# Excalibur1224/Cuda-v-MPI

Hardware: AMD Instinct MI355X
Metric: Riemann subintervals/sec at N=1e9 fp64; |error| vs analytic π (higher is better)
Workload: dtype fp64

## Files before the change

csrc/include/miint/integrands.hpp:

```cpp
#pragma once

#include <hip/hip_runtime.h>

#include "miint/common.hpp"
#include "miint/fast_trig.hpp"

namespace miint {

template <class D>
struct TileDefaults {
  template <DivMode M>
  __host__ __device__ static constexpr int tile_len() { return 32; }
  template <int U, DivMode M>
  __device__ static constexpr double anchor() { return 0.0; }
  template <int U, DivMode M>
  __device__ __forceinline__ double tile_acc(double x0, double h, double acc) const {
    return acc + static_cast<const D*>(this)->template tile<U, M>(x0, h);
  }
};

struct Pi4 : TileDefaults<Pi4> {
  static constexpr double kScale = 4.0;
  static constexpr int kPairs = 16;
  static constexpr int kSub = 2 * kPairs;
  static constexpr int kSubs = 12;
  static constexpr int kSeriesTile = kSub * kSubs;
  static constexpr double kSumK2 = (kSeriesTile / 2) * (kSeriesTile / 2 - 1) * (kSeriesTile - 1) / 3.0 +
                                   (kSeriesTile / 2) * (kSeriesTile / 2 - 1) + kSeriesTile / 4.0;
  static_assert(kSumK2 == 4718560.0, "sum of squared midpoint offsets of a 384-sample tile");

  template <DivMode M>
  __host__ __device__ static constexpr int tile_len() {
    return (M == DivMode::kSeries || M == DivMode::kSeriesExact) ? kSeriesTile : 32;
  }

  static constexpr double kMeanK2 = 85.25;
  static constexpr int kPk2Sgpr = 5;
  double pk[kPairs];
  double pk2[kPairs];
  double pc[kSubs / 2];
  double pcm[kSubs / 2];
  double c15;
  typedef float f32x2 __attribute__((ext_vector_type(2)));
  f32x2 pkf[kPairs];

  __device__ __forceinline__ static double opaque_s(double v) {
    asm volatile("" : "+s"(v));
    return v;
  }
  __device__ __forceinline__ static double opaque_v(double v) {
    asm volatile("" : "+v"(v));
    return v;
  }
  template <bool K2 = true>
  __device__ __forceinline__ void init() {
#pragma unroll
    for (int j = 0; j < kPairs; ++j) {
      pk[j] = opaque_s(j + 0.5);
      const double k2 = (j + 0.5) * (j + 0.5) - kMeanK2;
      if constexpr (K2) {
        pk2[j] = j < kPk2Sgpr ? opaque_s(k2) : opaque_v(k2);
      } else {
        pk2[j] = k2;
        const f32x2 kk = {j + 0.5f, -(j + 0.5f)};
        pkf[j] = __builtin_bit_cast(f32x2, opaque_s(__builtin_bit_cast(double, kk)));
      }
    }
#pragma unroll
    for (int i = 0; i < kSubs / 2; ++i) {
      const double c0 = kSub * (i + 0.5);
      pc[i] = opaque_s(c0);
      pcm[i] = opaque_s(c0 + kMeanK2 / c0);
    }
    c15 = opaque_s(1.5);
  }

  __device__ __forceinline__ double point(double x) const { return 1.0 / fma(x, x, 1.0); }

  __device__ __forceinline__ static double recip_narrow(double d) {
    double r = __builtin_amdgcn_rcp(d);
    r = fma(r, fma(-d, r, 1.0), r);
    r = fma(r, fma(-d, r, 1.0), r);
    return fma(fma(-d, r, 1.0), r, r);
  }

  struct Seed {
    double s, em, a, b;
  };
  __device__ __forceinline__ static Seed seed(double xm, double h) {
    const double dm = fma(xm, xm, 1.0);
    double s = __builtin_amdgcn_rcp(dm);
    s = fma(s, fma(-dm, s, 1.0), s);
    return {s, fma(-dm, s, 1.0), (-2.0 * h) * xm * s, -(h * h) * s};
  }
  __device__ __forceinline__ Seed seed_half(double xm, double h) const {
    const double dm = fma(xm, xm, 1.0);
    const double s = __builtin_amdgcn_rcp(dm);
    return {s, fma(-dm, s, c15), (-2.0 * h) * xm * s, -(h * h) * s};
  }
  __device__ __forceinline__ static double side(const double* t, int q) {
    return q < kSubs / 2 ? -t[kSubs / 2 - 1 - q] : t[q - kSubs / 2];
  }
  __device__ __forceinline__ double centre_g(const Seed& sd, int q) const {
    return fma(side(pc, q), fma(side(pcm, q), sd.b, sd.a), sd.em);
  }
  __device__ __forceinline__ double centre_slope(const Seed& sd, double b2, int q) const {
    return fma(side(pc, q), b2, sd.a);
  }

  template <int U, DivMode M>
  __device__ __forceinline__ double tile(double x0, double h) const {
    static_assert(U % 2 == 0, "pair evaluation needs an even tile");
    static_assert(M != DivMode::kSeries, "kSeries runs through tile_acc");
    if constexpr (M == DivMode::kIeee) {
      double acc = 0.0;
#pragma unroll
      for (int u = 0; u < U; ++u) {
        const double x = fma(static_cast<double>(u), h, x0);
        acc += recip_narrow(fma(x, x, 1.0));
      }
      return acc;
    } else {
      const Seed sd = seed(fma(0.5 * (U - 1), h, x0), h);
      double t1a = 0.0, t1b = 0.0, t2 = 0.0;
#pragma unroll
      for (int u = 0; u < U; u += 2) {
        const double xa = fma(static_cast<double>(u), h, x0);
        const double xb = fma(static_cast<double>(u + 1), h, x0);
        const double ea = fma(-fma(xa, xa, 1.0), sd.s, 1.0);
        const double eb = fma(-fma(xb, xb, 1.0), sd.s, 1.0);
        t1a += ea;
        t1b += eb;
        t2 = fma(ea, ea, t2);
        t2 = fma(eb, eb, t2);
      }
      return fma(sd.s, (t1a + t1b) + t2, static_cast<double>(U) * sd.s);
    }
  }

  template <int U, DivMode M>
  __device__ static constexpr double anchor() {
    return (M == DivMode::kSeries || M == DivMode::kSeriesExact) ? 0.5 * (U - 1) : 0.0;
  }

  __device__ __forceinline__ Seed seed_exact(double xm, double h) const {
    const double dm = fma(xm, xm, 1.0);
    const double s = __builtin_amdgcn_rcp(dm);
    const double q = xm * s;
    const double qe = fma(xm, s, -q);
    const double em = fma(-xm, qe, fma(-xm, q, 1.0 - s));
    return {s, em, (-2.0 * h) * xm * s, -(h * h) * s};
  }

  template <int U, DivMode M>
  __device__ __forceinline__ double tile_acc(double xa, double h, double acc) const {
    if constexpr (M == DivMode::kSeries) {
      static_assert(U == kSeriesTile, "series tiles are kSubs sub-tiles of kSub samples");
      const Seed sd = seed_half(xa, h);
      const double b2 = 2.0 * sd.b;
      double t = 0.75 * U;
#pragma unroll
      for (int q = 0; q < kSubs; ++q) {
        const double eh = centre_g(sd, q);
        const double a = centre_slope(sd, b2, q);
#pragma unroll
        for (int j = 0; j < kPairs; ++j) {
          const double c = fma(pk2[j], sd.b, eh);
          const double gp = fma(pk[j], a, c);
          const double gn = fma(-pk[j], a, c);
          t = fma(gp, gp, t);
          t = fma(gn, gn, t);
          asm volatile("" : "+v"(t));
        }
      }
      return fma(sd.s, t, acc);
    } else if constexpr (M == DivMode::kSeriesExact) {
      static_assert(U == kSeriesTile, "series tiles are kSubs sub-tiles of kSub samples");
      const Seed sd = seed_exact(xa, h);
      const double b2 = 2.0 * sd.b;
      const double lin = fma(kSumK2, sd.b, static_cast<double>(U) * sd.em);
      f32x2 t2 = {0.0f, 0.0f};
#pragma unroll
      for (int q = 0; q < kSubs; ++q) {
        const f32x2 ec = static_cast<float>(centre_g(sd, q));
        const f32x2 a = static_cast<float>(centre_slope(sd, b2, q));
#pragma unroll
        for (int j = 0; j < kPairs; ++j) {
          const f32x2 e = __builtin_elementwise_fma(pkf[j], a, ec);
          t2 = __builtin_elementwise_fma(e, e, t2);
          asm volatile("" : "+v"(t2));
        }
      }
      const double t = lin + (static_cast<double>(t2.x) + static_cast<double>(t2.y));
      return fma(sd.s, t, fma(sd.s, static_cast<double>(U), acc));
    } else {
      return acc + tile<U, M>(xa, h);
    }
  }

  __device__ __forceinline__ double series_exact_point(double xm, double h, int u) const {
    const Seed sd = seed_exact(xm, h);
    const double b2 = 2.0 * sd.b;
    const int q = u / kSub, w = u % kSub;
    const double ec = centre_g(sd, q);
    const double a = centre_slope(sd, b2, q);
    const int j = w >= kSub / 2 ? w - kSub / 2 : kSub / 2 - 1 - w;
    const double kj = w >= kSub / 2 ? pk[j] : -pk[j];
    const double e = fma(kj, a, fma(fma(kj, kj, -kMeanK2), sd.b, ec));
    const float e_sq = fmaf(static_cast<float>(kj), static_cast<float>(a), static_cast<float>(ec));
    const float sq = e_sq * e_sq;
    return fma(sd.s, e + static_cast<double>(sq), sd.s);
  }

  __device__ __forceinline__ double series_point(double xm, double h, int u) const {
    const Seed sd = seed_half(xm, h);
    const double b2 = 2.0 * sd.b;
    const int q = u / kSub, w = u % kSub;
    const double eh = centre_g(sd, q);
    const double a = centre_slope(sd, b2, q);
    const int j = w >= kSub / 2 ? w - kSub / 2 : kSub / 2 - 1 - w;
    const double c = fma(pk2[j], sd.b, eh);
    const double g = w >= kSub / 2 ? fma(pk[j], a, c) : fma(-pk[j], a, c);
    return sd.s * fma(g, g, 0.75);
  }
};

struct Pi4Wide : TileDefaults<Pi4Wide> {
  static constexpr double kScale = 4.0;
  __device__ __forceinline__ double point(double x) const { return 1.0 / fma(x, x, 1.0); }
  template <int U, DivMode M>
  __device__ __forceinline__ double tile(double x0, double h) const {
    static_assert(M == DivMode::kIeee, "wide-domain Pi4 runs IEEE division only");
    double acc = 0.0;
#pragma unroll
    for (int u = 0; u < U; ++u) acc += point(fma(static_cast<double>(u), h, x0));
    return acc;
  }
};
constexpr double kPi4NarrowMaxX = 0x1p249;

__device__ __forceinline__ void tile_sincos(double th, double& S, double& C) {
  constexpr double kTwoOverPi = 6.36619772367581382433e-01;
  constexpr double kPio2Hi = 1.57079632673412561417e+00;
  constexpr double kPio2Lo = 6.07710050650619224932e-11;
  const double n = rint(th * kTwoOverPi);
  const double r = fma(-n, kPio2Lo, fma(-n, kPio2Hi, th));
  const int q = static_cast<int>(n);
  const double z = r * r, w = z * z;
  const double s26 = fma(z, fma(z, fma(z, fma(z, 1.58969099521155010221e-10,
                                                -2.50507602534068634195e-08),
                                           2.75573137070700676789e-06),
                                      -1.98412698298579493134e-04),
                         8.33333333332248946124e-03);
  const double sr = fma(r * z, fma(z, s26, -1.66666666666666324348e-01), r);
  const double c13 = fma(z, fma(z, 2.48015872894767294178e-05, -1.38888888888741095749e-03),
                         4.16666666666666019037e-02);
  const double c46 = fma(z, fma(z, -1.13596475577881948265e-11, 2.08757232129817482790e-09),
                         -2.75573143513906633035e-07);
  const double rc = fma(w * w, c46, z * c13);
  const double hz = 0.5 * z, cw = 1.0 - hz;
  const double cc = cw + (((1.0 - cw) - hz) + z * rc);
  const bool swap = (q & 1) != 0;
  const double a = swap ? cc : sr, b = swap ? sr : cc;
  S = (q & 2) ? -a : a;
  C = ((q + 1) & 2) ? -b : b;
}

template <int Subs>
struct AngleSeries {
  static constexpr int kPairs = 8;
  static constexpr int kSub = 2 * kPairs;
  static constexpr int kSubs = Subs;
  static constexpr int kSeriesTile = kSub * kSubs;
  static_assert(2 * kPairs + kSubs <= kSinTrig, "RiemannParams::trig layout");
  double ck[kPairs], sk[kPairs];
  double cc[kSubs / 2], sc[kSubs / 2];

  __device__ __forceinline__ void init_trig(const double* trig) {
#pragma unroll
    for (int j = 0; j < kPairs; ++j) {
      ck[j] = trig[j];
      sk[j] = trig[kPairs + j];
    }
#pragma unroll
    for (int i = 0; i < kSubs / 2; ++i) {
      cc[i] = trig[2 * kPairs + 2 * i];
      sc[i] = trig[2 * kPairs + 2 * i + 1];
    }
  }
  __device__ __forceinline__ void centre(double S, double C, int q, double& Sq,
                                         double& Cq) const {
    const int i = q < kSubs / 2 ? kSubs / 2 - 1 - q : q - kSubs / 2;
    const double c = cc[i], s = q < kSubs / 2 ? -sc[i] : sc[i];
    Sq = fma(C, s, S * c);
    Cq = fma(-S, s, C * c);
  }
  template <bool COS>
  __device__ __forceinline__ double tile_sum(double theta_m) const {
    double S, C;
    tile_sincos(theta_m, S, C);
    double t = 0.0;
#pragma unroll
    for (int q = 0; q < kSubs; ++q) {
      double Sq, Cq;
      centre(S, C, q, Sq, Cq);
      const double base = COS ? Cq : Sq, side = COS ? -Sq : Cq;
#pragma unroll
      for (int j = 0; j < kPairs; ++j) {
        const double u = base * ck[j];
        t += fma(side, sk[j], u);
        t += fma(-side, sk[j], u);
        asm volatile("" : "+v"(t));
      }
    }
    return t;
  }
  template <bool COS>
  __device__ __forceinline__ double point_of(double theta_m, int u) const {
    double S, C, Sq, Cq;
    tile_sincos(theta_m, S, C);
    const int q = u / kSub, w = u % kSub;
    centre(S, C, q, Sq, Cq);
    const double base = COS ? Cq : Sq, side = COS ? -Sq : Cq;
    const int j = w >= kSub / 2 ? w - kSub / 2 : kSub / 2 - 1 - w;
    const double v = base * ck[j];
    return w >= kSub / 2 ? fma(side, sk[j], v) : fma(-side, sk[j], v);
  }
};

template <int U, int SHIFT, class ANGLE, class LIB>
__device__ __forceinline__ double trig_tile_sum(double x0, double h, const ANGLE& angle,
                                                const LIB& lib) {
  TrigTile q;
  if (trig_tile(angle(x0), angle(fma(static_cast<double>(U - 1), h, x0)), SHIFT, q)) {
    double a0 = 0.0, a1 = 0.0;
    if (q.use_cos) {
#pragma unroll
      for (int u = 0; u < U; u += 2) {
        a0 += trig_sample<true>(angle(fma(static_cast<double>(u), h, x0)), q);
        a1 += trig_sample<true>(angle(fma(static_cast<double>(u + 1), h, x0)), q);
      }
    } else {
#pragma unroll
      for (int u = 0; u < U; u += 2) {
        a0 += trig_sample<false>(angle(fma(static_cast<double>(u), h, x0)), q);
        a1 += trig_sample<false>(angle(fma(static_cast<double>(u + 1), h, x0)), q);
      }
    }
    const double t = a0 + a1;
    return q.neg ? -t : t;
  }
  double acc0 = 0.0, acc1 = 0.0;
#pragma unroll 1
  for (int u = 0; u < U; u += 2) {
    acc0 += lib(angle(fma(static_cast<double>(u), h, x0)));
    acc1 += lib(angle(fma(static_cast<double>(u + 1), h, x0)));
  }
  return acc0 + acc1;
}
template <int U, int SHIFT, class ANGLE, class LIB>
__device__ __forceinline__ double trig_tile_point(double x0, double h, int u, const ANGLE& angle,
                                                  const LIB& lib) {
  TrigTile q;
  const double th = angle(fma(static_cast<double>(u), h, x0));
  if (!trig_tile(angle(x0), angle(fma(static_cast<double>(U - 1), h, x0)), SHIFT, q))
    return lib(th);
  const double v = q.use_cos ? trig_sample<true>(th, q) : trig_sample<false>(th, q);
  return q.neg ? -v : v;
}
struct IdentityAngle {
  __device__ __forceinline__ double operator()(double x) const { return x; }
};
struct ScaledAngle {
  double k;
  __device__ __forceinline__ double operator()(double x) const { return x * k; }
};
struct OcmlSin {
  __device__ __forceinline__ double operator()(double x) const { return sin(x); }
};
struct OcmlCos {
  __device__ __forceinline__ double operator()(double x) const { return cos(x); }
};

struct Sin : TileDefaults<Sin>, AngleSeries<12> {
  static constexpr double kScale = 1.0;
  template <DivMode M>
  __host__ __device__ static constexpr int tile_len() {
    return M == DivMode::kSeries ? kSeriesTile : 32;
  }
  template <int U, DivMode M>
  __device__ static constexpr double anchor() {
    return M == DivMode::kSeries ? 0.5 * (U - 1) : 0.0;
  }
  __device__ __forceinline__ void init(const double* trig) { init_trig(trig); }
  __device__ __forceinline__ double point(double x) const { return sin(x); }
  template <int U, DivMode M>
  __device__ __forceinline__ double tile_acc(double xa, double h, double acc) const {
    if constexpr (M == DivMode::kSeries) {
      static_assert(U == kSeriesTile, "angle series tiles are kSeriesTile samples");
      return acc + tile_sum<false>(xa);
    } else {
      return acc + tile<U, M>(xa, h);
    }
  }
  __device__ __forceinline__ double series_point(double xm, int u) const {
    return point_of<false>(xm, u);
  }
  template <int U, DivMode>
  __device__ __forceinline__ double tile(double x0, double h) const {
    return trig_tile_sum<U, 0>(x0, h, IdentityAngle{}, OcmlSin{});
  }
  template <int U>
  __device__ __forceinline__ double ieee_point(double x0, double h, int u) const {
    return trig_tile_point<U, 0>(x0, h, u, IdentityAngle{}, OcmlSin{});
  }
};
struct SinLib : Sin {
  template <int U, DivMode>
  __device__ __forceinline__ double tile(double x0, double h) const {
    double acc0 = 0.0, acc1 = 0.0;
#pragma unroll 1
    for (int u = 0; u < U; u += 2) {
      acc0 += sin(fma(static_cast<double>(u), h, x0));
      acc1 += sin(fma(static_cast<double>(u + 1), h, x0));
    }
    return acc0 + acc1;
  }
  template <int U, DivMode M>
  __device__ __forceinline__ double tile_acc(double xa, double h, double acc) const {
    static_assert(M != DivMode::kSeries, "SinLib is the kIeee reference");
    return acc + tile<U, M>(xa, h);
  }
  template <int U>
  __device__ __forceinline__ double ieee_point(double x0, double h, int u) const {
    return sin(fma(static_cast<double>(u), h, x0));
  }
};

template <int NC>
struct Poly : TileDefaults<Poly<NC>> {
  static constexpr double kScale = 1.0;
  static constexpr int kPairs = 16;
  static constexpr int kSub = 2 * kPairs;
  static constexpr int kSubs = 2;
  static constexpr int kSeriesTile = kSub * kSubs;
  double c[NC];
  double cs[NC];
  double pk[kPairs];
  double c16;
  double inv_h;

  __device__ __forceinline__ void init(const double* coef, int n) {
#pragma unroll
    for (int k = 0; k < NC; ++k) c[k] = k < n ? coef[k] : 0.0;
  }
  __device__ __forceinline__ void init_series(const double* coef_h, int n, double h) {
#pragma unroll
    for (int k = 0; k < NC; ++k) cs[k] = k < n ? coef_h[k] : 0.0;
#pragma unroll
    for (int j = 0; j < kPairs; ++j) {
      double v = j + 0.5;
      asm volatile("" : "+s"(v));
      pk[j] = v;
    }
    double v = 0.5 * kSub;
    asm volatile("" : "+s"(v));
    c16 = v;
    inv_h = 1.0 / h;
  }
  template <DivMode M>
  __host__ __device__ static constexpr int tile_len() {
    return M == DivMode::kSeries ? kSeriesTile : 32;
  }
  template <int U, DivMode M>
  __device__ static constexpr double anchor() {
    return M == DivMode::kSeries ? 0.5 * (U - 1) : 0.0;
  }
  __device__ __forceinline__ double point(double x) const {
    double r = c[NC - 1];
#pragma unroll
    for (int k = NC - 2; k >= 0; --k) r = fma(r, x, c[k]);
    return r;
  }
  template <int U, DivMode>
  __device__ __forceinline__ double tile(double x0, double h) const {
    double acc = 0.0;
#pragma unroll 4
    for (int u = 0; u < U; ++u) acc += point(fma(static_cast<double>(u), h, x0));
    return acc;
  }
  __device__ __forceinline__ void shift(double uc, double (&b)[NC]) const {
#pragma unroll
    for (int i = 0; i < NC; ++i) b[i] = cs[i];
#pragma unroll
    for (int m = 0; m < NC - 1; ++m)
#pragma unroll
      for (int i = NC - 2; i >= m; --i) b[i] = fma(b[i + 1], uc, b[i]);
  }
  __device__ __forceinline__ void parts(const double (&b)[NC], double K, double& E,
                                        double& O) const {
    constexpr int ev = (NC - 1) & ~1, od = ((NC - 2) | 1);
    E = b[ev];
#pragma unroll
    for (int e = ev - 2; e >= 0; e -= 2) E = fma(E, K, b[e]);
    O = b[od];
#pragma unroll
    for (int o = od - 2; o >= 1; o -= 2) O = fma(O, K, b[o]);
  }
  template <int U, DivMode M>
  __device__ __forceinline__ double tile_acc(double xm, double h, double acc) const {
    if constexpr (M == DivMode::kSeries) {
      static_assert(U == kSeriesTile && NC <= 8, "Taylor-pair tiles: NC <= 8, 64 samples");
      const double um = xm * inv_h;
      double t = 0.0;
#pragma unroll
      for (int q = 0; q < kSubs; ++q) {
        double b[NC];
        shift(um + (q == 0 ? -c16 : c16), b);
#pragma unroll
        for (int j = 0; j < kPairs; ++j) {
          double E, O;
          parts(b, pk[j] * pk[j], E, O);
          t += fma(pk[j], O, E);
          t += fma(-pk[j], O, E);
          asm volatile("" : "+v"(t));
        }
      }
      return acc + t;
    } else {
      return acc + tile<U, M>(xm, h);
    }
  }
  __device__ __forceinline__ double series_point(double xm, int u) const {
    const int q = u / kSub, w = u % kSub;
    double b[NC];
    shift(xm * inv_h + (q == 0 ? -c16 : c16), b);
    const int j = w >= kSub / 2 ? w - kSub / 2 : kSub / 2 - 1 - w;
    double E, O;
    parts(b, pk[j] * pk[j], E, O);
    return w >= kSub / 2 ? fma(pk[j], O, E) : fma(-pk[j], O, E);
  }
};

struct TrainVel : TileDefaults<TrainVel>, AngleSeries<8> {
  double inv_ts, vs;
  static constexpr double kScale = 1.0;
  template <DivMode M>
  __host__ __device__ static constexpr int tile_len() {
    return M == DivMode::kSeries ? kSeriesTile : 32;
  }
  template <int U, DivMode M>
  __device__ static constexpr double anchor() {
    return M == DivMode::kSeries ? 0.5 * (U - 1) : 0.0;
  }
  __device__ __forceinline__ double point(double t) const {
    return (1.0 - cos(t * inv_ts)) * vs;
  }
  template <int U, DivMode M>
  __device__ __forceinline__ double tile_acc(double ta, double h, double acc) const {
    if constexpr (M == DivMode::kSeries) {
      static_assert(U == kSeriesTile, "angle series tiles are kSeriesTile samples");
      return fma(-vs, tile_sum<true>(ta * inv_ts), fma(vs, static_cast<double>(U), acc));
    } else {
      return acc + tile<U, M>(ta, h);
    }
  }
  __device__ __forceinline__ double series_point(double tm, int u) const {
    return (1.0 - point_of<true>(tm * inv_ts, u)) * vs;
  }
  template <int U, DivMode>
  __device__ __forceinline__ double tile(double x0, double h) const {
    const double c = trig_tile_sum<U, 1>(x0, h, ScaledAngle{inv_ts}, OcmlCos{});
    return fma(-vs, c, vs * static_cast<double>(U));
  }
  template <int U>
  __device__ __forceinline__ double ieee_point(double x0, double h, int u) const {
    return (1.0 - trig_tile_point<U, 1>(x0, h, u, ScaledAngle{inv_ts}, OcmlCos{})) * vs;
  }
};
struct TrainVelLib : TrainVel {
  template <int U, DivMode>
  __device__ __forceinline__ double tile(double x0, double h) const {
    double acc0 = 0.0, acc1 = 0.0;
#pragma unroll 1
    for (int u = 0; u < U; u += 2) {
      acc0 += point(fma(static_cast<double>(u), h, x0));
      acc1 += point(fma(static_cast<double>(u + 1), h, x0));
    }
    return acc0 + acc1;
  }
  template <int U, DivMode M>
  __device__ __forceinline__ double tile_acc(double xa, double h, double acc) const {
    static_assert(M != DivMode::kSeries, "TrainVelLib is the kIeee reference");
    return acc + tile<U, M>(xa, h);
  }
  template <int U>
  __device__ __forceinline__ double ieee_point(double x0, double h, int u) const {
    return point(fma(static_cast<double>(u), h, x0));
  }
};

struct Table : TileDefaults<Table> {
  const double* lds;
  int nseg;
  static constexpr double kScale = 1.0;
  static constexpr int kPairs = 16;
  static constexpr int kSub = 2 * kPairs;
  static constexpr int kSubs = 2;
  static constexpr int kSeriesTile = kSub * kSubs;
  double pk[kPairs];
  double c16;
  double hspan;
  double inv_h;

  __device__ __forceinline__ static double opaque_s(double v) {
    asm volatile("" : "+s"(v));
    return v;
  }
  __device__ __forceinline__ void init() {
#pragma unroll
    for (int j = 0; j < kPairs; ++j) pk[j] = opaque_s(j + 0.5);
    c16 = opaque_s(0.5 * kSub);
    hspan = opaque_s(0.5 * (kSeriesTile - 1));
  }
  template <DivMode M>
  __host__ __device__ static constexpr int tile_len() {
    return M == DivMode::kSeries ? kSeriesTile : 32;
  }
  template <int U, DivMode M>
  __device__ static constexpr double anchor() {
    return M == DivMode::kSeries ? 0.5 * (U - 1) : 0.0;
  }
  __device__ __forceinline__ int segment(double t) const {
    return static_cast<int>(fmin(fmax(t, 0.0), static_cast<double>(nseg - 1)));
  }
  __device__ __forceinline__ double point(double t) const {
    const int i = segment(t);
    const double fr = t - static_cast<double>(i);
    const double v0 = lds[i];
    const double v1 = lds[i + 1];
    return fma(v1 - v0, fr, v0);
  }
  template <int U, DivMode>
  __device__ __forceinline__ double tile(double x0, double h) const {
    double acc0 = 0.0, acc1 = 0.0;
#pragma unroll
    for (int u = 0; u < U; u += 2) {
      acc0 += point(fma(static_cast<double>(u), h, x0));
      acc1 += point(fma(static_cast<double>(u + 1), h, x0));
    }
    return acc0 + acc1;
  }
  __device__ __forceinline__ void ends(double xm, double h, int& lo, int& hi) const {
    lo = segment(fma(-hspan, h, xm));
    hi = segment(fma(hspan, h, xm));
  }
  __device__ __forceinline__ void line(double xm, double h, int i, double& vm, double& D) const {
    const double v0 = lds[i];
    const double d = lds[i + 1] - v0;
    vm = fma(d, xm - static_cast<double>(i), v0);
    D = d * h;
  }
  struct Kink {
    double dD, kk;
  };
  __device__ __forceinline__ Kink kink(double xm, double h, int lo, double& vm, double& D) const {
    const double v0 = lds[lo], v1 = lds[lo + 1], v2 = lds[lo + 2];
    const double d0 = v1 - v0;
    vm = fma(d0, xm - static_cast<double>(lo), v0);
    D = d0 * h;
    return {((v2 - v1) - d0) * h, (static_cast<double>(lo + 1) - xm) * inv_h};
  }
  template <bool KINK>
  __device__ __forceinline__ double line_sum(double vm, double D, const Kink& kn) const {
    double t = 0.0;
#pragma unroll
    for (int q = 0; q < kSubs; ++q) {
      const double c0 = q == 0 ? -c16 : c16;
      const double vc = fma(c0, D, vm);
      const double r = c0 - kn.kk;
#pragma unroll
      for (int j = 0; j < kPairs; ++j) {
        double gp = fma(pk[j], D, vc);
        double gn = fma(-pk[j], D, vc);
        if constexpr (KINK) {
          gp = fma(fmax(r + pk[j], 0.0), kn.dD, gp);
          gn = fma(fmax(r - pk[j], 0.0), kn.dD, gn);
        }
        t += gp;
        t += gn;
        asm volatile("" : "+v"(t));
      }
    }
    return t;
  }
  template <int U, DivMode M>
  __device__ __forceinline__ double tile_acc(double xm, double h, double acc) const {
    if constexpr (M == DivMode::kSeries) {
      static_assert(U == kSeriesTile, "segment tiles are kSubs sub-tiles of kSub samples");
      int lo, hi;
      ends(xm, h, lo, hi);
      double vm, D;
      if (lo == hi) {
        line(xm, h, lo, vm, D);
        return acc + line_sum<false>(vm, D, Kink{0.0, 0.0});
      }
      if (hi == lo + 1) {
        const Kink kn = kink(xm, h, lo, vm, D);
        return acc + line_sum<true>(vm, D, kn);
      }
      const double x0 = fma(-hspan, h, xm);
      double s0 = 0.0, s1 = 0.0;
#pragma unroll 1
      for (int u = 0; u < U; u += 2) {
        s0 += point(fma(static_cast<double>(u), h, x0));
        s1 += point(fma(static_cast<double>(u + 1), h, x0));
      }
      return acc + (s0 + s1);
    } else {
      return acc + tile<U, M>(xm, h);
    }
  }
  __device__ __forceinline__ double series_point(double xm, double h, int u) const {
    int lo, hi;
    ends(xm, h, lo, hi);
    if (hi > lo + 1) return point(fma(static_cast<double>(u), h, fma(-hspan, h, xm)));
    double vm, D;
    Kink kn{0.0, 0.0};
    if (lo == hi) line(xm, h, lo, vm, D);
    else kn = kink(xm, h, lo, vm, D);
    const int q = u / kSub, w = u % kSub;
    const double c0 = q == 0 ? -c16 : c16;
    const double vc = fma(c0, D, vm);
    const double r = c0 - kn.kk;
    const int j = w >= kSub / 2 ? w - kSub / 2 : kSub / 2 - 1 - w;
    double g = w >= kSub / 2 ? fma(pk[j], D, vc) : fma(-pk[j], D, vc);
    if (lo != hi) g = fma(fmax(w >= kSub / 2 ? r + pk[j] : r - pk[j], 0.0), kn.dD, g);
    return g;
  }
};

}
```

Before: 28180 billion.

## Compute sub-tile centres in packed fp32 and hand-schedule pair FMAs in asm

Moves the per-sub-tile centre value and slope computation of the exact series mode from fp64 to packed fp32. Each packed op now yields the mirrored ± sub-tile pair together. The inner 16-pair loop is replaced by inline assembly of v_pk_fma_f32 with op_sel operand selection and two independent accumulators, which shortens the dependency chain and avoids broadcasting scalars. The aim is to cut fp64 work and accumulator latency in the hot loop. The cost is lower precision in the centre terms and brittle hand-written asm that is tied to 16 pairs.

```diff
diff --git a/csrc/include/miint/integrands.hpp b/csrc/include/miint/integrands.hpp
--- a/csrc/include/miint/integrands.hpp
+++ b/csrc/include/miint/integrands.hpp
@@ -42,7 +42,12 @@
   double pcm[kSubs / 2];
   double c15;
   typedef float f32x2 __attribute__((ext_vector_type(2)));
+#ifndef MIINT_PI4_PAIR_ORDER
+#define MIINT_PI4_PAIR_ORDER 1
+#endif
   f32x2 pkf[kPairs];
+  f32x2 pcf[kSubs / 2];
+  f32x2 pcmf[kSubs / 2];
 
   __device__ __forceinline__ static double opaque_s(double v) {
     asm volatile("" : "+s"(v));
@@ -71,6 +76,12 @@
       const double c0 = kSub * (i + 0.5);
       pc[i] = opaque_s(c0);
       pcm[i] = opaque_s(c0 + kMeanK2 / c0);
+      if constexpr (!K2) {
+        const float c0f = static_cast<float>(c0), cmf = static_cast<float>(c0 + kMeanK2 / c0);
+        const f32x2 cc = {c0f, -c0f}, cm = {cmf, -cmf};
+        pcf[i] = __builtin_bit_cast(f32x2, opaque_s(__builtin_bit_cast(double, cc)));
+        pcmf[i] = __builtin_bit_cast(f32x2, opaque_s(__builtin_bit_cast(double, cm)));
+      }
     }
     c15 = opaque_s(1.5);
   }
@@ -149,8 +160,66 @@
     const double q = xm * s;
     const double qe = fma(xm, s, -q);
     const double em = fma(-xm, qe, fma(-xm, q, 1.0 - s));
-    return {s, em, (-2.0 * h) * xm * s, -(h * h) * s};
-  }
+    return {s, em, (-2.0 * h) * q, -(h * h) * s};
+  }
+  struct SeedF32 {
+    float em, a, b, b2;
+  };
+  __device__ __forceinline__ static SeedF32 seed_f32(const Seed& sd) {
+    const float b = static_cast<float>(sd.b);
+    return {static_cast<float>(sd.em), static_cast<float>(sd.a), b, b + b};
+  }
+  __device__ __forceinline__ f32x2 centres_f32(const SeedF32& sf, int i) const {
+    const f32x2 in = __builtin_elementwise_fma(pcmf[i], f32x2{sf.b, sf.b}, f32x2{sf.a, sf.a});
+    return __builtin_elementwise_fma(pcf[i], in, f32x2{sf.em, sf.em});
+  }
+  __device__ __forceinline__ f32x2 slopes_f32(const SeedF32& sf, int i) const {
+    return __builtin_elementwise_fma(pcf[i], f32x2{sf.b2, sf.b2}, f32x2{sf.a, sf.a});
+  }
+
+#define MIINT_PAIRS2(K0, K1, SEL, TA, TB)                         \
+  "v_pk_fma_f32 %[e0], %[" K0 "], %[a], %[c]" SEL "\n\t"         \
+  "v_pk_fma_f32 %[e1], %[" K1 "], %[a], %[c]" SEL "\n\t"         \
+  "v_pk_fma_f32 %[ta], %[e0], %[e0], " TA "\n\t"                 \
+  "v_pk_fma_f32 %[tb], %[e1], %[e1], " TB "\n\t"
+#define MIINT_SUBTILE(SEL, TA0, TB0)                                                  \
+  MIINT_PAIRS2("k0", "k1", SEL, TA0, TB0) MIINT_PAIRS2("k2", "k3", SEL, "%[ta]", "%[tb]")       \
+  MIINT_PAIRS2("k4", "k5", SEL, "%[ta]", "%[tb]") MIINT_PAIRS2("k6", "k7", SEL, "%[ta]", "%[tb]")   \
+  MIINT_PAIRS2("k8", "k9", SEL, "%[ta]", "%[tb]") MIINT_PAIRS2("k10", "k11", SEL, "%[ta]", "%[tb]") \
+  MIINT_PAIRS2("k12", "k13", SEL, "%[ta]", "%[tb]") MIINT_PAIRS2("k14", "k15", SEL, "%[ta]", "%[tb]")
+#define MIINT_SUBTILE_IN                                                                      \
+  [k0] "s"(pkf[0]), [k1] "s"(pkf[1]), [k2] "s"(pkf[2]), [k3] "s"(pkf[3]), [k4] "s"(pkf[4]),   \
+  [k5] "s"(pkf[5]), [k6] "s"(pkf[6]), [k7] "s"(pkf[7]), [k8] "s"(pkf[8]), [k9] "s"(pkf[9]),   \
+  [k10] "s"(pkf[10]), [k11] "s"(pkf[11]), [k12] "s"(pkf[12]), [k13] "s"(pkf[13]),             \
+  [k14] "s"(pkf[14]), [k15] "s"(pkf[15]), [a] "v"(a), [c] "v"(c)
+#define MIINT_SEL_LO " op_sel_hi:[1,0,0]"
+#define MIINT_SEL_HI " op_sel:[0,1,1]"
+#define MIINT_ZERO "0 op_sel_hi:[1,1,0]"
+  template <bool Hi, bool First>
+  __device__ __forceinline__ void subtile_squares(f32x2& ta, f32x2& tb, f32x2 a, f32x2 c) const {
+    static_assert(kPairs == 16, "the statement names 16 pair constants");
+    f32x2 e0, e1;
+    if constexpr (First) {
+      static_assert(Hi, "a tile starts with the sub-tile at -176");
+      asm volatile(MIINT_SUBTILE(MIINT_SEL_HI, MIINT_ZERO, MIINT_ZERO)
+                   : [e0] "=&v"(e0), [e1] "=&v"(e1), [ta] "=&v"(ta), [tb] "=&v"(tb)
+                   : MIINT_SUBTILE_IN);
+    } else if constexpr (Hi) {
+      asm volatile(MIINT_SUBTILE(MIINT_SEL_HI, "%[ta]", "%[tb]")
+                   : [e0] "=&v"(e0), [e1] "=&v"(e1), [ta] "+v"(ta), [tb] "+v"(tb)
+                   : MIINT_SUBTILE_IN);
+    } else {
+      asm volatile(MIINT_SUBTILE(MIINT_SEL_LO, "%[ta]", "%[tb]")
+                   : [e0] "=&v"(e0), [e1] "=&v"(e1), [ta] "+v"(ta), [tb] "+v"(tb)
+                   : MIINT_SUBTILE_IN);
+    }
+  }
+#undef MIINT_PAIRS2
+#undef MIINT_SUBTILE
+#undef MIINT_SUBTILE_IN
+#undef MIINT_SEL_LO
+#undef MIINT_SEL_HI
+#undef MIINT_ZERO
 
   template <int U, DivMode M>
   __device__ __forceinline__ double tile_acc(double xa, double h, double acc) const {
@@ -177,13 +246,35 @@
     } else if constexpr (M == DivMode::kSeriesExact) {
       static_assert(U == kSeriesTile, "series tiles are kSubs sub-tiles of kSub samples");
       const Seed sd = seed_exact(xa, h);
-      const double b2 = 2.0 * sd.b;
       const double lin = fma(kSumK2, sd.b, static_cast<double>(U) * sd.em);
+      const SeedF32 sf = seed_f32(sd);
       f32x2 t2 = {0.0f, 0.0f};
+      f32x2 ecs[kSubs / 2], aqs[kSubs / 2];
+#if MIINT_PI4_PAIR_ORDER
+      f32x2 tb;
 #pragma unroll
       for (int q = 0; q < kSubs; ++q) {
-        const f32x2 ec = static_cast<float>(centre_g(sd, q));
-        const f32x2 a = static_cast<float>(centre_slope(sd, b2, q));
+        const int i = q < kSubs / 2 ? kSubs / 2 - 1 - q : q - kSubs / 2;
+        if (q < kSubs / 2) {
+          ecs[i] = centres_f32(sf, i);
+          aqs[i] = slopes_f32(sf, i);
+        }
+        if (q == 0) subtile_squares<true, true>(t2, tb, aqs[i], ecs[i]);
+        else if (q < kSubs / 2) subtile_squares<true, false>(t2, tb, aqs[i], ecs[i]);
+        else subtile_squares<false, false>(t2, tb, aqs[i], ecs[i]);
+      }
+      t2 += tb;
+#else
+#pragma unroll
+      for (int q = 0; q < kSubs; ++q) {
+        const int i = q < kSubs / 2 ? kSubs / 2 - 1 - q : q - kSubs / 2;
+        if (q < kSubs / 2) {
+          ecs[i] = centres_f32(sf, i);
+          aqs[i] = slopes_f32(sf, i);
+        }
+        const float ecq = q < kSubs / 2 ? ecs[i].y : ecs[i].x;
+        const float aq = q < kSubs / 2 ? aqs[i].y : aqs[i].x;
+        const f32x2 ec = {ecq, ecq}, a = {aq, aq};
 #pragma unroll
         for (int j = 0; j < kPairs; ++j) {
           const f32x2 e = __builtin_elementwise_fma(pkf[j], a, ec);
@@ -191,6 +282,7 @@
           asm volatile("" : "+v"(t2));
         }
       }
+#endif
       const double t = lin + (static_cast<double>(t2.x) + static_cast<double>(t2.y));
       return fma(sd.s, t, fma(sd.s, static_cast<double>(U), acc));
     } else {
@@ -207,7 +299,11 @@
     const int j = w >= kSub / 2 ? w - kSub / 2 : kSub / 2 - 1 - w;
     const double kj = w >= kSub / 2 ? pk[j] : -pk[j];
     const double e = fma(kj, a, fma(fma(kj, kj, -kMeanK2), sd.b, ec));
-    const float e_sq = fmaf(static_cast<float>(kj), static_cast<float>(a), static_cast<float>(ec));
+    const SeedF32 sf = seed_f32(sd);
+    const int i = q < kSubs / 2 ? kSubs / 2 - 1 - q : q - kSubs / 2;
+    const f32x2 ecs = centres_f32(sf, i), aqs = slopes_f32(sf, i);
+    const float e_sq = fmaf(static_cast<float>(kj), q < kSubs / 2 ? aqs.y : aqs.x,
+                            q < kSubs / 2 ? ecs.y : ecs.x);
     const float sq = e_sq * e_sq;
     return fma(sd.s, e + static_cast<double>(sq), sd.s);
   }
```

Result: faster. 31310 billion (median of 6 runs) (+11.1%).
